# intel/QATzip

Hardware: AMD Instinct MI355X
Metric: compress + decompress GB/s (input bytes), QZ_DEFLATE_GZIP_EXT L1, 64 KB chunks (higher is better)
Workload: dtype u8

## Files before the change

### qatzip_amd/csrc/qzk_common.h

```cpp
#ifndef QZK_COMMON_H
#define QZK_COMMON_H
#include <stdint.h>

#ifdef QZ_SIM
#include "hipsim.h"
#define QZ_DEV static inline
#define QZ_KERNEL static void
#define QZ_KERNEL_MAX(n) static void
#define QZ_KERNEL_OCC(n, w) static void
#define QZ_LDS static
#define QZ_CONST static const
#else
#include <hip/hip_runtime.h>
#define QZ_DEV static __device__ __forceinline__
#define QZ_KERNEL static __global__ void
#define QZ_KERNEL_MAX(n) static __global__ void __launch_bounds__(n)
#define QZ_KERNEL_OCC(n, w) static __global__ void __launch_bounds__(n, w)
#define QZ_LDS __shared__
#define QZ_CONST static __device__ const

QZ_DEV uint64_t qz_ballot(bool p) { return __ballot(p); }
QZ_DEV uint32_t qz_shfl(uint32_t v, int src) { return (uint32_t)__shfl((int)v, src, 64); }
QZ_DEV uint32_t qz_readlane(uint32_t v, int src) { return (uint32_t)__builtin_amdgcn_readlane((int)v, src); }
QZ_DEV uint32_t qz_readfirstlane(uint32_t v) { return (uint32_t)__builtin_amdgcn_readfirstlane((int)v); }
QZ_DEV uint32_t qz_writelane(uint32_t old, uint32_t val, int sel) { return (int)(threadIdx.x & 63) == sel ? val : old; }
QZ_DEV void qz_wave_sync()
{
    __builtin_amdgcn_fence(__ATOMIC_RELEASE, "workgroup");
    __builtin_amdgcn_wave_barrier();
    __builtin_amdgcn_fence(__ATOMIC_ACQUIRE, "workgroup");
}
QZ_DEV void qz_lds_sync()
{
    __builtin_amdgcn_fence(__ATOMIC_ACQ_REL, "wavefront");
    __builtin_amdgcn_wave_barrier();
}
QZ_DEV void qz_block_sync() { __syncthreads(); }
QZ_DEV int qz_lane() { return (int)(threadIdx.x & 63); }
QZ_DEV uint8_t qz_ld8_l2(const uint8_t *p) { return __hip_atomic_load(p, __ATOMIC_RELAXED, __HIP_MEMORY_SCOPE_AGENT); }
#endif
#ifdef QZ_SIM
static inline void qz_lds_sync() { qz_wave_sync(); }
static inline uint32_t qz_writelane(uint32_t old, uint32_t val, int sel) { return qz_lane() == sel ? val : old; }
static inline uint8_t qz_ld8_l2(const uint8_t *p) { return *p; }
#endif

#ifndef QZ_SIM
QZ_DEV uint32_t qz_wave_incl_scan(uint32_t v)
{
    v += (uint32_t)__builtin_amdgcn_update_dpp(0, (int)v, 0x111, 0xf, 0xf, false);
    v += (uint32_t)__builtin_amdgcn_update_dpp(0, (int)v, 0x112, 0xf, 0xf, false);
    v += (uint32_t)__builtin_amdgcn_update_dpp(0, (int)v, 0x114, 0xf, 0xf, false);
    v += (uint32_t)__builtin_amdgcn_update_dpp(0, (int)v, 0x118, 0xf, 0xf, false);
    v += (uint32_t)__builtin_amdgcn_update_dpp(0, (int)v, 0x142, 0xa, 0xf, false);
    v += (uint32_t)__builtin_amdgcn_update_dpp(0, (int)v, 0x143, 0xc, 0xf, false);
    return v;
}
#else
static inline uint32_t qz_wave_incl_scan(uint32_t v)
{
    const int lane = qz_lane();
    for (int d = 1; d < 64; d <<= 1) {
        uint32_t o = qz_shfl(v, lane - d);
        if (lane >= d) v += o;
    }
    return v;
}
#endif

QZ_DEV int qz_popc64(uint64_t v) { return __builtin_popcountll(v); }
QZ_DEV int qz_ctz64(uint64_t v) { return __builtin_ctzll(v); }
QZ_DEV int qz_ctz32(uint32_t v) { return __builtin_ctz(v); }
QZ_DEV int qz_msb64(uint64_t v) { return 63 - __builtin_clzll(v); }
QZ_DEV uint64_t qz_below(int l) { return l >= 64 ? ~0ull : ((1ull << l) - 1); }

typedef struct __attribute__((packed, aligned(1))) { uint32_t v; } qz_u32u;
typedef struct __attribute__((packed, aligned(1))) { uint16_t v; } qz_u16u;
QZ_DEV uint32_t qz_ld32(const uint8_t *p) { return ((const qz_u32u *)p)->v; }
QZ_DEV uint32_t qz_ld16(const uint8_t *p) { return ((const qz_u16u *)p)->v; }

QZ_DEV uint32_t qz_uniform(uint32_t v) { return qz_readfirstlane(v); }

#endif
```

### qatzip_amd/csrc/qzk_deflate_lz77.h

```cpp
#ifndef QZK_DEFLATE_LZ77_H
#define QZK_DEFLATE_LZ77_H
#include "qzk_common.h"
#include "qzk_crcmath.h"

#define QZK_WSIZE 32768
#define QZK_MAXDIST 32506
#define QZK_MINLOOK 262
#define QZK_LITBUF 32767
#define QZK_MAXBLK 20
#define QZK_CAP 16
#define QZK_WLIM 61
#define QZK_NICE 8
#define QZK_MAXINS 4
#define QZK_HSIZE 65536
#ifndef QZK_CNBLOG
#define QZK_CNBLOG (-1)
#endif
#if QZK_CNBLOG >= 0
#define QZK_CNB (1 << QZK_CNBLOG)
#else
#define QZK_CNB 0
#endif
#ifndef QZK_PF
#define QZK_PF (QZK_CNB ? 1 : 0)
#endif
#ifndef QZK_PF_MINL
#define QZK_PF_MINL 30
#endif
#ifndef QZK_NSLOT
#define QZK_NSLOT 256
#endif
#ifndef QZK_RING
#define QZK_RING 4096
#endif
#ifndef QZK_K1_OCC
#define QZK_K1_OCC 5
#endif
#define QZK_RINGW (QZK_RING / 4)
#ifndef QZK_NSLOT2
#define QZK_NSLOT2 128
#endif
#ifndef QZK_NSLOT3
#if QZK_CNB
#define QZK_NSLOT3 0
#else
#define QZK_NSLOT3 128
#endif
#endif
#define QZK_K1_PARSEW (2 * QZK_NSLOT + QZK_RINGW + 4 + QZK_NSLOT2 + QZK_NSLOT3 + 3 * QZK_CNB)
#ifndef QZK_K1_WAVES
#define QZK_K1_WAVES 4
#endif

#ifndef QZK_K1_TABGRP
#define QZK_K1_TABGRP 5
#endif
#define QZK_K1_TABW (QZK_K1_WAVES * QZK_K1_TABGRP)
#define QZK_K1_TABROWS(wgs) ((((wgs) + 8u * QZK_K1_TABGRP - 1) / (8u * QZK_K1_TABGRP)) * 8u)

typedef struct __attribute__((aligned(16))) { uint32_t w0, w1, w2, ep; } qzk_bkt;
typedef uint32_t qzk_u32x4 __attribute__((vector_size(16)));

QZ_DEV qzk_u32x4 qzk_ld_bkt(const qzk_bkt *p)
{
#ifdef QZ_SIM
    return *(const qzk_u32x4 *)p;
#else
    qzk_u32x4 v;
    asm volatile("global_load_dwordx4 %0, %1, off sc1\n\ts_waitcnt vmcnt(0)" : "=v"(v) : "v"(p) : "memory");
    return v;
#endif
}

QZ_DEV void qzk_ld_bkt_ahead(qzk_u32x4 *v, const qzk_bkt *p)
{
#ifdef QZ_SIM
    *v = *(const qzk_u32x4 *)p;
#else
    asm volatile("global_load_dwordx4 %0, %1, off sc1" : "+v"(*v) : "v"(p) : "memory");
#endif
}
QZ_DEV void qzk_wait_ahead(qzk_u32x4 *v)
{
#ifdef QZ_SIM
    (void)v;
#else
    asm volatile("s_waitcnt vmcnt(0)" : "+v"(*v) : : "memory");
#endif
}

#ifdef QZ_SIM
static unsigned long qzk_sim_count[2];
#define QZK_SIMC(k) do { if (qz_lane() == 0) qzk_sim_count[k]++; } while (0)
#else
#define QZK_SIMC(k) do { } while (0)
#endif
#if defined(QZK_PROF) && !defined(QZ_SIM)
#define QZK_T(k) do { uint64_t t_ = __builtin_readcyclecounter(); prof[k] += t_ - tprev; tprev = t_; } while (0)
#define QZK_C(k, v) do { prof[k] += (uint64_t)(v); } while (0)
#else
#define QZK_T(k) do { } while (0)
#define QZK_C(k, v) do { } while (0)
#endif

typedef struct {
    uint32_t nsym;
    uint32_t nfull;
    uint32_t bstart[QZK_MAXBLK];
    uint32_t can_store;
    uint32_t n;
#ifdef QZK_PROF
    uint64_t prof[24];
#endif
} qzk_lzmeta;

#define QZK_CDESC_FINAL 0x80000000u
QZ_DEV uint32_t qzk_chunk_len(const uint32_t *cdesc, uint32_t chunk, uint64_t src_len, uint32_t chunk_sz)
{
    if (cdesc) return cdesc[chunk] & ~QZK_CDESC_FINAL;
    const uint64_t coff = (uint64_t)chunk * chunk_sz;
    return (uint32_t)((src_len - coff) < chunk_sz ? (src_len - coff) : chunk_sz);
}

QZ_DEV uint32_t qzk_ld32g(const uint8_t *src, uint64_t off, uint64_t src_len)
{
    if (off + 4 <= src_len) return qz_ld32(src + off);
    uint32_t v = 0;
    for (int k = 0; k < 4; k++) if (off + k < src_len) v |= (uint32_t)src[off + k] << (8 * k);
    return v;
}

QZ_DEV uint32_t qzk_ld32g_fast(const uint8_t *src, uint64_t off, uint64_t src_len)
{
    return off + 4 <= src_len ? qz_ld32(src + off) : qzk_ld32g(src, off, src_len);
}

QZ_DEV uint32_t qzk_alignbyte(uint32_t hi, uint32_t lo, uint32_t s)
{
#ifdef QZ_SIM
    return (uint32_t)((((uint64_t)hi << 32) | lo) >> (8 * s));
#else
    return __builtin_amdgcn_alignbyte(hi, lo, s);
#endif
}

QZ_DEV int qzk_wave_matchlen(const uint8_t *src, uint64_t src_len, uint64_t a, uint64_t b, int maxlen, int lane)
{
    for (int off = 0; off < maxlen; off += 256) {
        int o = off + 4 * lane;
        bool act = o < maxlen;
        uint32_t x = 0;
        if (act) x = qzk_ld32g(src, a + o, src_len) ^ qzk_ld32g(src, b + o, src_len);
        uint64_t mm = qz_ballot(act && x != 0);
        if (mm) {
            int f = qz_ctz64(mm);
            uint32_t xf = qz_readlane(x, f);
            int len = off + 4 * f + (qz_ctz32(xf) >> 3);
            return len < maxlen ? len : maxlen;
        }
    }
    return maxlen;
}

QZ_DEV void qzk_lz77_chunk(const uint8_t *src, uint64_t src_len, uint32_t chunk_sz, uint32_t chunk,
                           uint8_t *sym_lc, uint16_t *sym_dist, qzk_lzmeta *meta, qzk_bkt *tab, uint32_t epoch,
                           const uint32_t *cdesc, uint32_t *lds, const qzk_k1crc_lds *crcT, uint32_t *crc_slot)
{
    uint32_t *const slot = lds, *const scnt = lds + QZK_NSLOT, *const ring = lds + 2 * QZK_NSLOT, *const slot2 = ring + QZK_RINGW + 4;
    uint32_t *const slot3 = slot2 + QZK_NSLOT2; (void)slot3;
#if QZK_CNB
    uint32_t *const ctag = slot3 + QZK_NSLOT3, *const cpos = ctag + QZK_CNB;
#pragma nounroll
    for (uint32_t i = (uint32_t)qz_lane(); i < QZK_CNB; i += 64) ctag[i] = 0;
#endif
    uint32_t rhi = 0;
    uint32_t crc_acc = 0;
    uint32_t rnext = qzk_ld32g_fast(src, (uint64_t)chunk * chunk_sz + 4 * (uint32_t)qz_lane(), src_len);
#define QZK_RING16(dst, ca) do { const uint32_t r_ = (ca) & (QZK_RING - 1), i_ = r_ >> 2, s_ = r_ & 3; \
        const uint32_t d0_ = ring[i_], d1_ = ring[i_ + 1], d2_ = ring[i_ + 2], d3_ = ring[i_ + 3], d4_ = ring[i_ + 4]; \
        (dst)[0] = qzk_alignbyte(d1_, d0_, s_); (dst)[1] = qzk_alignbyte(d2_, d1_, s_); \
        (dst)[2] = qzk_alignbyte(d3_, d2_, s_); (dst)[3] = qzk_alignbyte(d4_, d3_, s_); } while (0)
#define QZK_RING4(ca) ({ const uint32_t r_ = (ca) & (QZK_RING - 1), i_ = r_ >> 2; \
        qzk_alignbyte(ring[i_ + 1], ring[i_], r_ & 3); })
#define QZK_AHEAD (64 + 258 + 6)

    const int lane = qz_lane();
    const uint64_t coff = (uint64_t)chunk * chunk_sz;
    const uint32_t n = qzk_chunk_len(cdesc, chunk, src_len, chunk_sz);
    uint8_t *olc = sym_lc;
    uint16_t *odist = sym_dist;
    qzk_lzmeta *mt = meta + chunk;
    auto wave_matchlen = [&](uint32_t ca, uint32_t cb, int maxlen) -> int {
        const bool near = (int64_t)cb >= (int64_t)rhi - QZK_RING;
        for (int off = 0; off < maxlen; off += 256) {
            const int o = off + 4 * lane;
            const bool act = o < maxlen;
            uint32_t x = 0;
            if (act) x = QZK_RING4(ca + (uint32_t)o) ^ (near ? QZK_RING4(cb + (uint32_t)o) : qzk_ld32g(src, coff + cb + (uint32_t)o, src_len));
            const uint64_t mm = qz_ballot(act && x != 0);
            if (mm) {
                const int f = qz_ctz64(mm);
                const uint32_t xf = qz_readlane(x, f);
                const int len = off + 4 * f + (qz_ctz32(xf) >> 3);
                return len < maxlen ? len : maxlen;
            }
        }
        return maxlen;
    };

    qz_lds_sync();

    uint32_t base = 0;
    uint32_t fill = n < 65536u ? n : 65536u;
    uint32_t avail_in = n - fill;
    uint32_t pos = 0;
    uint32_t nsym = 0, nfull = 0, cur_bstart = 0, can_store = 0;
    mt->bstart[0] = 0;
#if QZK_PF
    qzk_u32x4 pf = {0, 0, 0, 0};
    uint64_t pf_okm = 0;
    uint32_t pf_base = 0, pf_mark = 0, wcount = 0;
    bool pf_lost = false;
    uint64_t dPm = 0, dSTm = 0;
    uint32_t dnsym = 0, dv_sym = 0, dv_h = 0, dv_e0 = 0, dv_e1 = 0, dv_e2 = 0;
#define QZK_DEFERRED_STORES() do { \
        if ((dPm >> lane) & 1) { const uint32_t i_ = dnsym + (uint32_t)qz_popc64(dPm & qz_below(lane)); \
                                 olc[i_] = (uint8_t)dv_sym; odist[i_] = (uint16_t)(dv_sym >> 8); } \
        if ((dSTm >> lane) & 1) { const qzk_u32x4 e_ = {dv_e0, dv_e1, dv_e2, epoch}; *(qzk_u32x4 *)&tab[(size_t)dv_h * QZK_K1_TABW] = e_; } \
        dPm = 0; dSTm = 0; } while (0)
    bool pf_live = false;
#endif
#if defined(QZK_PROF) && !defined(QZ_SIM)
    uint64_t prof[24] = {0}; uint64_t tprev = __builtin_readcyclecounter();
#endif

    for (;;) {
        uint32_t look = fill - pos;
        if (look < QZK_MINLOOK) {
            if (pos - base >= (uint32_t)(QZK_WSIZE + QZK_MAXDIST)) {
                base += QZK_WSIZE;
#if QZK_CNB
                qz_lds_sync();
#pragma nounroll
                for (uint32_t i = (uint32_t)lane; i < 2 * QZK_CNB; i += 64) {
                    const uint32_t v = cpos[i];
                    const int a = (int)(v & 0xffffu) - QZK_WSIZE, b = (int)(v >> 16) - QZK_WSIZE;
                    cpos[i] = (uint32_t)(a > 0 ? a : 0) | (uint32_t)(b > 0 ? b : 0) << 16;
                }
                qz_lds_sync();
#endif
            }
            if (avail_in) {
                uint32_t more = 65536u - (fill - base);
                uint32_t rd = avail_in < more ? avail_in : more;
                fill += rd; avail_in -= rd;
            }
            look = fill - pos;
            if (look == 0) break;
        }

        QZK_T(0); QZK_C(8, 1);
#if QZK_PF
        qzk_wait_ahead(&pf);
        QZK_T(17);
        QZK_DEFERRED_STORES();
        QZK_T(18);
#endif
        const uint32_t B = pos - base;
        const uint32_t p = B + (uint32_t)lane;
        const uint32_t pa = pos + (uint32_t)lane;
        const int avail = pa < fill ? (int)(fill - pa) : 0;
        const bool canh = avail >= 3;
        const bool guard = coff + pos + 64 + 2 * QZK_CAP > src_len;
        uint32_t w0 = 0, w1 = 0, w2 = 0, w3 = 0;
        {
            if (rhi < pos + QZK_AHEAD) {
                do {
                    const uint32_t a = rhi + 4 * (uint32_t)lane;
                    const uint32_t ri = (a >> 2) & (QZK_RINGW - 1);
                    ring[ri] = rnext;
                    if (ri < 4) ring[ri + QZK_RINGW] = rnext;
                    if (crcT && a + 4 <= n) crc_acc = qzk_k1crc_step(crcT, crc_acc, rnext);
                    rhi += 256;
                    rnext = qzk_ld32g_fast(src, coff + a + 256, src_len);
                } while (rhi < pos + QZK_AHEAD);
                qz_lds_sync();
            }
            uint32_t w[4];
            QZK_RING16(w, pa);
            w0 = w[0]; w1 = w[1]; w2 = w[2]; w3 = w[3];
        }
        const uint32_t h = (((w0 & 0xf) << 12) ^ (((w0 >> 8) & 0xff) << 6) ^ ((w0 >> 16) & 0xff)) & 0xffff;
        const uint32_t bucket = h;
        const uint32_t key = h & (QZK_NSLOT - 1);

        int nvalid = look < 64 ? (int)look : 64;
        int lim = nvalid < QZK_WLIM ? nvalid : QZK_WLIM;
        {
            int lstop;
            int first_short = (int)look - (QZK_MINLOOK - 1);
            if (first_short < 0) first_short = 0;
            if (avail_in) lstop = first_short;
            else {
                int sl = (int)(QZK_WSIZE + QZK_MAXDIST) - (int)B;
                lstop = first_short > sl ? first_short : sl;
            }
            if (lstop < 1) lstop = 1;
            if (lim > lstop) lim = lstop;
        }
        QZK_T(1);
        qz_lds_sync();
        qzk_u32x4 ev = {0, 0, 0, 0};
#if QZK_CNB
        const uint32_t cset = ((h * 40503u) >> (16 - QZK_CNBLOG)) & (QZK_CNB - 1);
        const uint32_t ct = ctag[cset], cp0 = cpos[cset], cp1 = cpos[QZK_CNB + cset];
        const bool chit = canh && ct == (h | 0x10000u);
        QZK_C(8, (uint64_t)qz_popc64(qz_ballot(chit)) << 32);
#if QZK_PF
        bool evhave = false;
        int limdata = 64;
        {
            const uint32_t sh = pos - pf_base;
            if (pf_live && !pf_lost && sh < 64u - (QZK_PF_MINL + 3)) {
                const int sl = lane + (int)sh;
                const uint32_t a0 = qz_shfl(pf[0], sl), a1 = qz_shfl(pf[1], sl), a2 = qz_shfl(pf[2], sl), a3 = qz_shfl(pf[3], sl);
                if (canh && !chit && sl < 64 && ((pf_okm >> (sl & 63)) & 1) && slot[key] != (pf_mark | h) && scnt[(h >> 8) & (QZK_NSLOT - 1)] != (pf_mark | h)) {
                    ev[0] = a0; ev[1] = a1; ev[2] = a2; ev[3] = a3; evhave = true;
                }
            }
            const bool lack = canh && !chit && !evhave;
            const uint64_t LACK = qz_ballot(lack);
            if (LACK) {
                const int fl = qz_ctz64(LACK);
                if (fl < QZK_PF_MINL + 3) { if (lack) { ev = qzk_ld_bkt(&tab[(size_t)bucket * QZK_K1_TABW]); evhave = true; } QZK_C(15, 1ull << 32); QZK_SIMC(0); }
                else limdata = fl - 3;
            }
        }
#else
        const bool evhave = canh && !chit;
        if (canh && !chit) ev = qzk_ld_bkt(&tab[(size_t)bucket * QZK_K1_TABW]);
#endif
#if QZK_PF
        if (lim > limdata) lim = limdata;
        QZK_SIMC(1);
#endif
        QZK_T(16);
        const bool ev_ok = ev[3] == epoch;
        uint32_t q0 = ev_ok ? ev[0] & 0xffffffu : 0, q1 = ev_ok ? (ev[0] >> 24) | ((ev[1] & 0xffffu) << 8) : 0,
                 q2 = ev_ok ? (ev[1] >> 16) | ((ev[2] & 0xffu) << 16) : 0, q3 = ev_ok ? ev[2] >> 8 : 0;
        if (chit) {
            q0 = (cp0 & 0xffffu) ? base + (cp0 & 0xffffu) : 0; q1 = (cp0 >> 16) ? base + (cp0 >> 16) : 0;
            q2 = (cp1 & 0xffffu) ? base + (cp1 & 0xffffu) : 0; q3 = (cp1 >> 16) ? base + (cp1 >> 16) : 0;
        }
#else
        if (canh) ev = qzk_ld_bkt(&tab[(size_t)bucket * QZK_K1_TABW]);
        const bool ev_ok = ev[3] == epoch;
        const uint32_t q0 = ev_ok ? ev[0] & 0xffffffu : 0, q1 = ev_ok ? (ev[0] >> 24) | ((ev[1] & 0xffffu) << 8) : 0,
                       q2 = ev_ok ? (ev[1] >> 16) | ((ev[2] & 0xffu) << 16) : 0, q3 = ev_ok ? ev[2] >> 8 : 0;
#endif
        const uint32_t lo = base + (p > QZK_MAXDIST ? p - QZK_MAXDIST : 0);
        const int maxlen = avail < 258 ? avail : 258;
        const int nice = avail < QZK_NICE ? avail : QZK_NICE;
        int best_len = 2; uint32_t best_c = 0;
        int l0 = 0, l1 = 0, l2 = 0, l3 = 0;
        bool suspect;
        int nc; uint32_t c0, c1, c2, c3;
        {
            uint32_t x[4][4];
            const bool ok0 = canh && q0 > base && pa - q0 <= QZK_MAXDIST;
            const bool ok1 = ok0 && q1 > lo;
            const bool ok2 = ok1 && q2 > lo;
            const bool ok3 = ok2 && q3 > lo;
            c0 = ok0 ? q0 : pa; c1 = ok1 ? q1 : pa; c2 = ok2 ? q2 : pa; c3 = ok3 ? q3 : pa;
            QZK_RING16(x[0], c0); QZK_RING16(x[1], c1); QZK_RING16(x[2], c2); QZK_RING16(x[3], c3);
#define QZK_LDF(k, ck) do { const uint32_t ca_ = (ck); if ((int64_t)ca_ < (int64_t)rhi - QZK_RING) { const uint64_t g_ = coff + ca_; \
        if (!guard) { x[k][0] = qz_ld32(src + g_); x[k][1] = qz_ld32(src + g_ + 4); x[k][2] = qz_ld32(src + g_ + 8); x[k][3] = qz_ld32(src + g_ + 12); } \
        else { x[k][0] = qzk_ld32g(src, g_, src_len); x[k][1] = qzk_ld32g(src, g_ + 4, src_len); x[k][2] = qzk_ld32g(src, g_ + 8, src_len); x[k][3] = qzk_ld32g(src, g_ + 12, src_len); } } } while (0)
#ifndef QZK_EXP_NOFAR
            QZK_LDF(0, c0); QZK_LDF(1, c1); QZK_LDF(2, c2); QZK_LDF(3, c3);
#endif
#undef QZK_LDF
            nc = (int)ok0 + (int)ok1 + (int)ok2 + (int)ok3;
            QZK_T(2);
            const uint32_t key2 = (h >> (16 - 8)) & (QZK_NSLOT2 - 1);
#if QZK_NSLOT3
            const uint32_t key3 = ((h * 40503u) >> 12) & (QZK_NSLOT3 - 1);
            if (canh) slot3[key3] = 0xffffffffu;
#endif
            if (canh) { slot[key] = 0xffffffffu; scnt[key] = 0; slot2[key2] = 0xffffffffu; }
            qz_lds_sync();
            if (canh) { atomicMin(&slot[key], ((uint32_t)lane << 16) | h); atomicAdd(&scnt[key], 1u); atomicMin(&slot2[key2], (uint32_t)lane); }
#if QZK_NSLOT3
            if (canh) atomicMin(&slot3[key3], (uint32_t)lane);
#endif
            qz_lds_sync();
            {
                const uint32_t sv = canh ? slot[key] : 0, sc = canh ? scnt[key] : 0, s2 = canh ? slot2[key2] : 0;
                suspect = canh && (sv >> 16) != (uint32_t)lane && !(sc == 2 && (sv & 0xffff) != h) && s2 != (uint32_t)lane;
#if QZK_NSLOT3
                if (suspect && slot3[key3] == (uint32_t)lane) suspect = false;
#endif
            }
            bool done = false;
            for (int k = 0; k < 4; k++) {
                const uint32_t ck = k == 0 ? c0 : k == 1 ? c1 : k == 2 ? c2 : c3;
                int len = 0;
                if (k < nc) {
                    uint32_t d;
                    len = QZK_CAP;
                    d = w3 ^ x[k][3]; if (d) len = 12 + (qz_ctz32(d) >> 3);
                    d = w2 ^ x[k][2]; if (d) len = 8 + (qz_ctz32(d) >> 3);
                    d = w1 ^ x[k][1]; if (d) len = 4 + (qz_ctz32(d) >> 3);
                    d = w0 ^ x[k][0]; if (d) len = (qz_ctz32(d) >> 3);
                    if (len > maxlen) len = maxlen;
                    if (!done) {
                        if (len > best_len) { best_len = len; best_c = ck; }
                        if (len >= nice) done = true;
                    }
                }
                if (k == 0) l0 = len; else if (k == 1) l1 = len; else if (k == 2) l2 = len; else l3 = len;
            }
        }
        uint32_t mlen = best_len >= 3 ? (uint32_t)best_len : 0;
        uint32_t mdist = mlen ? pa - best_c : 0;
        const bool capped = (best_len == QZK_CAP) && (maxlen > QZK_CAP);
        const bool exact0 = nc > 0 && pa - c0 == QZK_MAXDIST;

        QZK_T(3);
        const uint64_t CANH = qz_ballot(canh);
        const uint64_t CAPM = qz_ballot(capped);
        const uint64_t CX = qz_ballot(suspect) | CAPM;
        const uint64_t NOLIT = qz_ballot(mlen != 0) | CX;

        QZK_T(4);
#if QZK_PF
        {
            pf_base = pos + (uint32_t)lim; pf_live = true;
            pf_mark = 0x80000000u | wcount << 16; wcount = (wcount + 1) & 0x7fffu;
            const uint32_t ppa = pf_base + (uint32_t)lane;
            const bool pcanh = ppa + 3 <= fill;
            const uint32_t pw = QZK_RING4(ppa);
            const uint32_t ph = (((pw & 0xf) << 12) ^ (((pw >> 8) & 0xff) << 6) ^ ((pw >> 16) & 0xff)) & 0xffff;
            const uint32_t ps = ((ph * 40503u) >> (16 - QZK_CNBLOG)) & (QZK_CNB - 1);
            const uint32_t pct = ctag[ps], pc0 = cpos[ps], pc1 = cpos[QZK_CNB + ps];
            const uint32_t g0 = (pc0 & 0xffffu) ? base + (pc0 & 0xffffu) : 0, g1 = (pc0 >> 16) ? base + (pc0 >> 16) : 0,
                           g2 = (pc1 & 0xffffu) ? base + (pc1 & 0xffffu) : 0, g3 = (pc1 >> 16) ? base + (pc1 >> 16) : 0;
            pf[0] = g0 | (g1 << 24); pf[1] = (g1 >> 8) | (g2 << 16); pf[2] = (g2 >> 16) | (g3 << 8); pf[3] = epoch;
            if (pcanh && pct != (ph | 0x10000u)) qzk_ld_bkt_ahead(&pf, &tab[(size_t)ph * QZK_K1_TABW]);
            pf_okm = qz_ballot(pcanh);
        }
#endif
        uint64_t Pm = 0;
        uint64_t SHm = qz_ballot(mlen >= 3 && mlen <= QZK_MAXINS && avail - (int)mlen >= 3), S4m = qz_ballot(mlen == 4);
        int l = 0;
        while (l < lim) {
            uint64_t cxr = CX >> l;
            int nextc = cxr ? l + qz_ctz64(cxr) : 64;
            int stop = nextc < lim ? nextc : lim;
            while (l < stop) {
                const uint64_t nl = (NOLIT | (1ull << 63)) >> l;
                int e = l + qz_ctz64(nl);
                if (e > stop) e = stop;
                const uint32_t ml = qz_readlane(mlen, e);
                const int isM = e < stop ? 1 : 0;
                Pm |= ((1ull << (e - l + isM)) - 1) << l;
                l = e + (isM ? (int)ml : 0);
            }
            if (l >= lim || l != nextc) continue;
            QZK_T(5); QZK_C(9, 1);
            {
                const uint32_t h_l = qz_readlane(h, l);
                const uint64_t earlier = qz_ballot(canh && h == h_l) & qz_below(l);
                const uint32_t ml_l = qz_readlane(mlen, l);
                if (earlier == 0 && !((CAPM >> l) & 1)) {
                    QZK_C(15, 1);
                    Pm |= 1ull << l;
                    l += ml_l ? (int)ml_l : 1;
                    QZK_T(6);
                    continue;
                }
                const int avail_l = (int)look - l;
                const int maxlen_l = avail_l < 258 ? avail_l : 258;
                const int nice_l = avail_l < QZK_NICE ? avail_l : QZK_NICE;
                int cnt = 0, bl = 2; uint32_t bd = 0; bool fin = false;
                bool had_intra = false;
                if (earlier) {
                    const uint64_t ps = Pm & SHm;
                    const uint64_t I = (Pm & CANH) | (ps << 1) | (ps << 2) | ((ps & S4m) << 3);
                    uint64_t Sh = earlier & I;
                    if (B == 0) Sh &= ~1ull;
                    had_intra = Sh != 0;
                    if (Sh) {
                        const uint32_t a0 = qz_readlane(w0, l), a1 = qz_readlane(w1, l), a2 = qz_readlane(w2, l), a3 = qz_readlane(w3, l);
                        while (Sh && cnt < 4 && !fin) {
                            int j = qz_msb64(Sh);
                            Sh &= ~(1ull << j);
                            int len = QZK_CAP;
                            {
                                uint32_t d;
                                d = a3 ^ qz_readlane(w3, j); if (d) len = 12 + (qz_ctz32(d) >> 3);
                                d = a2 ^ qz_readlane(w2, j); if (d) len = 8 + (qz_ctz32(d) >> 3);
                                d = a1 ^ qz_readlane(w1, j); if (d) len = 4 + (qz_ctz32(d) >> 3);
                                d = a0 ^ qz_readlane(w0, j); if (d) len = (qz_ctz32(d) >> 3);
                            }
                            if (len > maxlen_l) len = maxlen_l;
                            if (len == QZK_CAP && maxlen_l > QZK_CAP)
                                len = wave_matchlen(pos + (uint32_t)l, pos + (uint32_t)j, maxlen_l);
                            cnt++;
                            if (len > bl) { bl = len; bd = (uint32_t)(l - j); }
                            if (len >= nice_l) fin = true;
                        }
                    }
                }
                const int nc_l = (int)qz_readlane((uint32_t)nc, l);
                const bool ex_l = qz_readlane((uint32_t)exact0, l) != 0;
                if (!fin && !(had_intra && ex_l)) {
                    for (int k = 0; k < nc_l && cnt < 4 && !fin; k++) {
                        const uint32_t ck = qz_readlane(k == 0 ? c0 : k == 1 ? c1 : k == 2 ? c2 : c3, l);
                        int len = (int)qz_readlane((uint32_t)(k == 0 ? l0 : k == 1 ? l1 : k == 2 ? l2 : l3), l);
                        if (len == QZK_CAP && maxlen_l > QZK_CAP)
                            len = wave_matchlen(pos + (uint32_t)l, ck, maxlen_l);
                        cnt++;
                        if (len > bl) { bl = len; bd = (pos + (uint32_t)l) - ck; }
                        if (len >= nice_l) fin = true;
                    }
                }
                uint32_t nl = bl >= 3 ? (uint32_t)bl : 0;
                if (lane == l) { mlen = nl; mdist = nl ? bd : 0; }
                {
                    const uint64_t bit = 1ull << l;
                    SHm = (nl >= 3 && nl <= QZK_MAXINS && avail_l - (int)nl >= 3) ? SHm | bit : SHm & ~bit;
                    S4m = nl == 4 ? S4m | bit : S4m & ~bit;
                }
                Pm |= 1ull << l;
                l += nl ? (int)nl : 1;
            }
            QZK_T(6);
        }

        QZK_T(5);
        const uint64_t ps = Pm & SHm;
        const uint64_t I = (Pm & CANH) | (ps << 1) | (ps << 2) | ((ps & S4m) << 3);
        const bool isP = (Pm >> lane) & 1, isI = (I >> lane) & 1;

        const uint32_t rank = (uint32_t)qz_popc64(Pm & qz_below(lane));
        const uint32_t idx = nsym + rank;
        const uint32_t step = mlen ? mlen : 1;
        if (isP) {
#if QZK_PF
            dv_sym = (mlen ? mlen - 3 : (w0 & 0xff)) | mdist << 8;
#else
            olc[idx] = (uint8_t)(mlen ? mlen - 3 : (w0 & 0xff));
            odist[idx] = (uint16_t)mdist;
#endif
        }
        {
            const bool closes = isP && ((idx + 1) % QZK_LITBUF == 0);
            const uint64_t cm = qz_ballot(closes);
            if (cm) {
                int f = qz_ctz64(cm);
                uint32_t nb = qz_readlane(pa + step, f);
                if (cur_bstart >= base) can_store |= 1u << nfull;
                nfull++;
                cur_bstart = nb;
                if (nfull < QZK_MAXBLK) mt->bstart[nfull] = nb;
            }
        }
#if QZK_PF
        dPm = Pm; dnsym = nsym;
#endif
        nsym += (uint32_t)qz_popc64(Pm);

        QZK_T(7);
        uint32_t n0 = pa, n1 = q0, n2 = q1, n3 = q2;
        bool store = isI;
        {
            uint64_t todo = I & qz_ballot(suspect);
            QZK_C(10, qz_popc64(todo)); QZK_C(11, qz_popc64(Pm));
            while (todo) {
                const int j = qz_msb64(todo);
                uint32_t b_j = qz_readlane(bucket, j);
                const uint64_t same = qz_ballot(canh && bucket == b_j) & I;
                todo &= ~same;
                uint64_t mates = same & qz_below(j);
                uint32_t m1 = 0, m2 = 0, m3 = 0;
                int nf = 1;
                while (mates && nf < 4) {
                    const int m = qz_msb64(mates);
                    mates &= ~(1ull << m);
                    const uint32_t mp = pos + (uint32_t)m;
                    if (nf == 1) m1 = mp; else if (nf == 2) m2 = mp; else m3 = mp;
                    nf++;
                }
                if (lane == j) {
                    if (nf == 2) { n1 = m1; n2 = q0; n3 = q1; }
                    else if (nf == 3) { n1 = m1; n2 = m2; n3 = q0; }
                    else if (nf == 4) { n1 = m1; n2 = m2; n3 = m3; }
                }
                if (((same >> lane) & 1) && lane < j) store = false;
            }
        }
#if QZK_PF
        dSTm = qz_ballot(store); dv_h = bucket;
        dv_e0 = n0 | (n1 << 24); dv_e1 = (n1 >> 8) | (n2 << 16); dv_e2 = (n2 >> 16) | (n3 << 8);
#else
        if (store) {
            const qzk_u32x4 e = {n0 | (n1 << 24), (n1 >> 8) | (n2 << 16), (n2 >> 16) | (n3 << 8), epoch};
            *(qzk_u32x4 *)&tab[(size_t)bucket * QZK_K1_TABW] = e;
        }
#endif
#if QZK_CNB
        {
            const bool ralloc = evhave && !isI;
            const uint32_t mark = (store ? 0x20040u : 0x20000u) | (uint32_t)lane;
#if QZK_PF
            {
                const uint32_t mk = pf_mark | h, key3 = (h >> 8) & (QZK_NSLOT - 1);
                if (store) slot[key] = mk;
                qz_lds_sync();
                const bool second = store && slot[key] != mk;
                if (second) scnt[key3] = mk;
                qz_lds_sync();
                pf_lost = qz_ballot(second && scnt[key3] != mk) != 0;
            }
#endif
            if (ralloc) ctag[cset] = mark;
            qz_lds_sync();
            if (store) ctag[cset] = mark;
            qz_lds_sync();
            if ((store || ralloc) && ctag[cset] == mark) {
                const uint32_t e0 = store ? n0 : q0, e1 = store ? n1 : q1, e2 = store ? n2 : q2, e3 = store ? n3 : q3;
                const uint32_t r0 = e0 > base ? e0 - base : 0, r1 = e1 > base ? e1 - base : 0, r2 = e2 > base ? e2 - base : 0,
                               r3 = e3 > base ? e3 - base : 0;
                cpos[cset] = r0 | r1 << 16; cpos[QZK_CNB + cset] = r2 | r3 << 16;
                ctag[cset] = h | 0x10000u;
            }
        }
#endif
        pos += (uint32_t)l;
        QZK_T(12);
    }

#if QZK_PF
    qzk_wait_ahead(&pf);
    QZK_DEFERRED_STORES();
#undef QZK_DEFERRED_STORES
#endif
    if (crcT) {
        for (; rhi < n; rhi += 256) {
            const uint32_t a = rhi + 4 * (uint32_t)lane;
            if (a + 4 <= n) crc_acc = qzk_k1crc_step(crcT, crc_acc, rnext);
            rnext = qzk_ld32g_fast(src, coff + a + 256, src_len);
        }
        const uint32_t n4 = n & ~3u;
        const uint32_t mine = n4 > 4u * (uint32_t)lane ? (n4 - 4u * (uint32_t)lane + 252u) >> 8 : 0;
        uint32_t part = 0;
        if (mine) part = qzk_multmodp(qzk_x2nmodp(crcT->x2n, n4 - (4u * (uint32_t)lane + 4u + 256u * (mine - 1)), 3), crc_acc);
        for (int d = 32; d >= 1; d >>= 1) part ^= qz_shfl(part, lane ^ d);
        if (n & 3u) {
            uint32_t c = 0xffffffffu;
            for (uint32_t i = n4; i < n; i++) c = qzk_crc_byte(c, src[coff + i]);
            part = qzk_multmodp(qzk_x2nmodp(crcT->x2n, n & 3u, 3), part) ^ ~c;
        }
        *crc_slot = part;
    }
    if (cur_bstart >= base) can_store |= 1u << nfull;
    mt->nsym = nsym; mt->nfull = nfull; mt->can_store = can_store; mt->n = n;
#if defined(QZK_PROF) && !defined(QZ_SIM)
    for (int k = 0; k < 24; k++) mt->prof[k] = prof[k];
#endif
#undef QZK_RING16
#undef QZK_RING4
}

#endif
```

Before: 66.28.

## Streamline LZ77 candidate loads: unguarded far reads, batched ring reads, early-skip far loads

Far-window candidate reads now use one unaligned 16-byte load relative to the chunk base instead of guarded per-word loads, on the premise that the positions are always inside the already-seen input. Ring LDS reads for all four candidates are issued together before the byte-align step so their latencies overlap. Far loads for candidates 1-3 are skipped when candidate 0 already gives a nice-length match from the ring. The hash-slot LDS writes and atomics are made unconditional to remove divergence; this can disturb slots with values from lanes that cannot hash, and it drops the src_len bounds checks.

New measurement: 65.43. -1.3%, worse.

```diff
diff --git a/qatzip_amd/csrc/qzk_common.h b/qatzip_amd/csrc/qzk_common.h
--- a/qatzip_amd/csrc/qzk_common.h
+++ b/qatzip_amd/csrc/qzk_common.h
@@ -76,6 +76,7 @@
 
 typedef struct __attribute__((packed, aligned(1))) { uint32_t v; } qz_u32u;
 typedef struct __attribute__((packed, aligned(1))) { uint16_t v; } qz_u16u;
+typedef struct __attribute__((packed, aligned(1))) { uint32_t v[4]; } qz_u32x4u;
 QZ_DEV uint32_t qz_ld32(const uint8_t *p) { return ((const qz_u32u *)p)->v; }
 QZ_DEV uint32_t qz_ld16(const uint8_t *p) { return ((const qz_u16u *)p)->v; }
 
diff --git a/qatzip_amd/csrc/qzk_deflate_lz77.h b/qatzip_amd/csrc/qzk_deflate_lz77.h
--- a/qatzip_amd/csrc/qzk_deflate_lz77.h
+++ b/qatzip_amd/csrc/qzk_deflate_lz77.h
@@ -2,6 +2,9 @@
 #define QZK_DEFLATE_LZ77_H
 #include "qzk_common.h"
 #include "qzk_crcmath.h"
+#ifdef QZ_SIM
+#include <assert.h>
+#endif
 
 #define QZK_WSIZE 32768
 #define QZK_MAXDIST 32506
@@ -98,6 +101,9 @@
 #if defined(QZK_PROF) && !defined(QZ_SIM)
 #define QZK_T(k) do { uint64_t t_ = __builtin_readcyclecounter(); prof[k] += t_ - tprev; tprev = t_; } while (0)
 #define QZK_C(k, v) do { prof[k] += (uint64_t)(v); } while (0)
+#elif defined(QZK_ISA_MARKS) && !defined(QZ_SIM)
+#define QZK_T(k) asm volatile("; QZK_MARK " #k)
+#define QZK_C(k, v) do { } while (0)
 #else
 #define QZK_T(k) do { } while (0)
 #define QZK_C(k, v) do { } while (0)
@@ -180,23 +186,36 @@
         const uint32_t d0_ = ring[i_], d1_ = ring[i_ + 1], d2_ = ring[i_ + 2], d3_ = ring[i_ + 3], d4_ = ring[i_ + 4]; \
         (dst)[0] = qzk_alignbyte(d1_, d0_, s_); (dst)[1] = qzk_alignbyte(d2_, d1_, s_); \
         (dst)[2] = qzk_alignbyte(d3_, d2_, s_); (dst)[3] = qzk_alignbyte(d4_, d3_, s_); } while (0)
+#define QZK_RING16_RD(raw, ca) do { const uint32_t i_ = ((ca) & (QZK_RING - 1)) >> 2; \
+        (raw)[0] = ring[i_]; (raw)[1] = ring[i_ + 1]; (raw)[2] = ring[i_ + 2]; (raw)[3] = ring[i_ + 3]; (raw)[4] = ring[i_ + 4]; } while (0)
+#define QZK_RING16_AL(dst, raw, ca) do { const uint32_t s_ = (ca) & 3; \
+        (dst)[0] = qzk_alignbyte((raw)[1], (raw)[0], s_); (dst)[1] = qzk_alignbyte((raw)[2], (raw)[1], s_); \
+        (dst)[2] = qzk_alignbyte((raw)[3], (raw)[2], s_); (dst)[3] = qzk_alignbyte((raw)[4], (raw)[3], s_); } while (0)
 #define QZK_RING4(ca) ({ const uint32_t r_ = (ca) & (QZK_RING - 1), i_ = r_ >> 2; \
         qzk_alignbyte(ring[i_ + 1], ring[i_], r_ & 3); })
 #define QZK_AHEAD (64 + 258 + 6)
 
     const int lane = qz_lane();
     const uint64_t coff = (uint64_t)chunk * chunk_sz;
+    uint32_t pos = 0;
+    const uint8_t *const csrc = src + coff;
+#ifdef QZ_SIM
+#define QZK_FAR_OK(ca, len) assert((ca) + (len) <= pos && pos <= n && coff + n <= src_len)
+#else
+#define QZK_FAR_OK(ca, len) do { } while (0)
+#endif
+#define QZK_FAR32(ca) ({ const uint32_t f_ = (ca); QZK_FAR_OK(f_, 4u); qz_ld32(csrc + f_); })
     const uint32_t n = qzk_chunk_len(cdesc, chunk, src_len, chunk_sz);
     uint8_t *olc = sym_lc;
     uint16_t *odist = sym_dist;
     qzk_lzmeta *mt = meta + chunk;
     auto wave_matchlen = [&](uint32_t ca, uint32_t cb, int maxlen) -> int {
-        const bool near = (int64_t)cb >= (int64_t)rhi - QZK_RING;
+        const bool near = rhi - cb <= (uint32_t)QZK_RING;
         for (int off = 0; off < maxlen; off += 256) {
             const int o = off + 4 * lane;
             const bool act = o < maxlen;
             uint32_t x = 0;
-            if (act) x = QZK_RING4(ca + (uint32_t)o) ^ (near ? QZK_RING4(cb + (uint32_t)o) : qzk_ld32g(src, coff + cb + (uint32_t)o, src_len));
+            if (act) x = QZK_RING4(ca + (uint32_t)o) ^ (near ? QZK_RING4(cb + (uint32_t)o) : QZK_FAR32(cb + (uint32_t)o));
             const uint64_t mm = qz_ballot(act && x != 0);
             if (mm) {
                 const int f = qz_ctz64(mm);
@@ -213,7 +232,6 @@
     uint32_t base = 0;
     uint32_t fill = n < 65536u ? n : 65536u;
     uint32_t avail_in = n - fill;
-    uint32_t pos = 0;
     uint32_t nsym = 0, nfull = 0, cur_bstart = 0, can_store = 0;
     mt->bstart[0] = 0;
 #if QZK_PF
@@ -271,7 +289,6 @@
         const uint32_t pa = pos + (uint32_t)lane;
         const int avail = pa < fill ? (int)(fill - pa) : 0;
         const bool canh = avail >= 3;
-        const bool guard = coff + pos + 64 + 2 * QZK_CAP > src_len;
         uint32_t w0 = 0, w1 = 0, w2 = 0, w3 = 0;
         {
             if (rhi < pos + QZK_AHEAD) {
@@ -372,12 +389,30 @@
             const bool ok2 = ok1 && q2 > lo;
             const bool ok3 = ok2 && q3 > lo;
             c0 = ok0 ? q0 : pa; c1 = ok1 ? q1 : pa; c2 = ok2 ? q2 : pa; c3 = ok3 ? q3 : pa;
-            QZK_RING16(x[0], c0); QZK_RING16(x[1], c1); QZK_RING16(x[2], c2); QZK_RING16(x[3], c3);
-#define QZK_LDF(k, ck) do { const uint32_t ca_ = (ck); if ((int64_t)ca_ < (int64_t)rhi - QZK_RING) { const uint64_t g_ = coff + ca_; \
-        if (!guard) { x[k][0] = qz_ld32(src + g_); x[k][1] = qz_ld32(src + g_ + 4); x[k][2] = qz_ld32(src + g_ + 8); x[k][3] = qz_ld32(src + g_ + 12); } \
-        else { x[k][0] = qzk_ld32g(src, g_, src_len); x[k][1] = qzk_ld32g(src, g_ + 4, src_len); x[k][2] = qzk_ld32g(src, g_ + 8, src_len); x[k][3] = qzk_ld32g(src, g_ + 12, src_len); } } } while (0)
+            {
+                uint32_t r[4][5];
+                QZK_RING16_RD(r[0], c0); QZK_RING16_RD(r[1], c1); QZK_RING16_RD(r[2], c2); QZK_RING16_RD(r[3], c3);
+#ifndef QZ_SIM
+                asm volatile("" : : "v"(r[0][0]), "v"(r[0][1]), "v"(r[0][2]), "v"(r[0][3]), "v"(r[0][4]), "v"(r[1][0]), "v"(r[1][1]), "v"(r[1][2]), "v"(r[1][3]), "v"(r[1][4]),
+                                    "v"(r[2][0]), "v"(r[2][1]), "v"(r[2][2]), "v"(r[2][3]), "v"(r[2][4]), "v"(r[3][0]), "v"(r[3][1]), "v"(r[3][2]), "v"(r[3][3]), "v"(r[3][4]));
+#endif
+                QZK_RING16_AL(x[0], r[0], c0); QZK_RING16_AL(x[1], r[1], c1); QZK_RING16_AL(x[2], r[2], c2); QZK_RING16_AL(x[3], r[3], c3);
+            }
+#define QZK_LDF(k, ck) do { const uint32_t ca_ = (ck); if (rhi - ca_ > (uint32_t)QZK_RING) { QZK_FAR_OK(ca_, 16u); \
+        const qz_u32x4u f_ = *(const qz_u32x4u *)(csrc + ca_); x[k][0] = f_.v[0]; x[k][1] = f_.v[1]; x[k][2] = f_.v[2]; x[k][3] = f_.v[3]; } } while (0)
 #ifndef QZK_EXP_NOFAR
-            QZK_LDF(0, c0); QZK_LDF(1, c1); QZK_LDF(2, c2); QZK_LDF(3, c3);
+            bool older = true;
+            if (rhi - c0 <= (uint32_t)QZK_RING) {
+                int e = QZK_CAP;
+                uint32_t d;
+                d = w3 ^ x[0][3]; if (d) e = 12 + (qz_ctz32(d) >> 3);
+                d = w2 ^ x[0][2]; if (d) e = 8 + (qz_ctz32(d) >> 3);
+                d = w1 ^ x[0][1]; if (d) e = 4 + (qz_ctz32(d) >> 3);
+                d = w0 ^ x[0][0]; if (d) e = (qz_ctz32(d) >> 3);
+                older = !(ok0 && (e < maxlen ? e : maxlen) >= nice);
+            }
+            QZK_LDF(0, c0);
+            if (older) { QZK_LDF(1, c1); QZK_LDF(2, c2); QZK_LDF(3, c3); }
 #endif
 #undef QZK_LDF
             nc = (int)ok0 + (int)ok1 + (int)ok2 + (int)ok3;
@@ -385,20 +420,21 @@
             const uint32_t key2 = (h >> (16 - 8)) & (QZK_NSLOT2 - 1);
 #if QZK_NSLOT3
             const uint32_t key3 = ((h * 40503u) >> 12) & (QZK_NSLOT3 - 1);
-            if (canh) slot3[key3] = 0xffffffffu;
-#endif
-            if (canh) { slot[key] = 0xffffffffu; scnt[key] = 0; slot2[key2] = 0xffffffffu; }
+            slot3[key3] = 0xffffffffu;
+#endif
+            slot[key] = 0xffffffffu; scnt[key] = 0; slot2[key2] = 0xffffffffu;
             qz_lds_sync();
-            if (canh) { atomicMin(&slot[key], ((uint32_t)lane << 16) | h); atomicAdd(&scnt[key], 1u); atomicMin(&slot2[key2], (uint32_t)lane); }
+            atomicMin(&slot[key], ((uint32_t)lane << 16) | h); atomicAdd(&scnt[key], 1u); atomicMin(&slot2[key2], (uint32_t)lane);
 #if QZK_NSLOT3
-            if (canh) atomicMin(&slot3[key3], (uint32_t)lane);
+            atomicMin(&slot3[key3], (uint32_t)lane);
 #endif
             qz_lds_sync();
             {
-                const uint32_t sv = canh ? slot[key] : 0, sc = canh ? scnt[key] : 0, s2 = canh ? slot2[key2] : 0;
+                const uint32_t sv = slot[key], sc = scnt[key], s2 = slot2[key2];
                 suspect = canh && (sv >> 16) != (uint32_t)lane && !(sc == 2 && (sv & 0xffff) != h) && s2 != (uint32_t)lane;
 #if QZK_NSLOT3
-                if (suspect && slot3[key3] == (uint32_t)lane) suspect = false;
+                const uint32_t s3 = slot3[key3];
+                suspect = suspect && s3 != (uint32_t)lane;
 #endif
             }
             bool done = false;
@@ -670,7 +706,11 @@
     for (int k = 0; k < 24; k++) mt->prof[k] = prof[k];
 #endif
 #undef QZK_RING16
+#undef QZK_RING16_RD
+#undef QZK_RING16_AL
 #undef QZK_RING4
-}
-
-#endif
+#undef QZK_FAR32
+#undef QZK_FAR_OK
+}
+
+#endif
```
